# dansarie/sboxgates

Measured on NVIDIA H100. Metric: candidate 3-LUT tuples/sec on rijndael.txt --lut (T-units + C-units per second), higher is better.
Workload: dtype u32 bitwise (LOP3)

## Files before the change

### include/sboxgates_b200.h

```cpp
#ifndef SBOXGATES_B200_H
#define SBOXGATES_B200_H

#include <stdint.h>

#ifdef __cplusplus
extern "C" {
#endif

#define SBG_OK 0
#define SBG_ERR_ARG (-1)
#define SBG_ERR_CUDA (-2)
#define SBG_ERR_OVERFLOW (-3)
#define SBG_ERR_STATE (-4)

#define SBG_MAX_GATES 500
#define SBG_LIST_CAP 100000
#define SBG_KEY_NONE UINT64_MAX
#define SBG_PROBLEM_SLOTS 64
#define SBG_LANES 8

typedef struct sbg_handle sbg_handle;

typedef struct {
  int32_t found;
// ... 87 lines not shown
int sbg_enum7(sbg_handle *h, int part, int nparts, const uint8_t *outer_order,
    const uint8_t *middle_order, uint64_t max_matches, sbg_match *out, uint64_t *n_out,
    uint64_t *total, uint64_t *feasible);
int sbg_enum3(sbg_handle *h, int part, int nparts, const uint16_t *gate_order,
    uint64_t max_matches, sbg_match *out, uint64_t *n_out, uint64_t *total, uint64_t *feasible);

int sbg_enum_fetch(sbg_handle *h, uint64_t first, uint64_t count, sbg_match *out, uint64_t *n_out);
int sbg_enum_pick(sbg_handle *h, const uint64_t *ranks, uint64_t nranks, sbg_match *out);

int sbg_enum_block_sums(sbg_handle *h, uint64_t *out, uint64_t *nblocks);
int sbg_enum_set_global(sbg_handle *h, const uint64_t *sums, uint64_t stride,
    const uint64_t *counts, int nparts, uint64_t *total);

#define SBG_MAX_DEPTH 1020
#define SBG_DEPTH_BINS 1024
int sbg_enum_set_depth(sbg_handle *h, const uint16_t *depth, int n, uint32_t max_depth);
int sbg_enum_depth_counts(sbg_handle *h, uint64_t *out, uint32_t nbins);

int sbg_plan_tickets(int width, int prefix_gates, int n, uint32_t excluded, int mode,
                     uint64_t waves, uint64_t *out);

#define SBG_WEIGHTED_ROW 76
int sbg_weighted_tickets(int n, uint32_t group_pairs, uint32_t *out);

int sbg_ordering_row(int width, int k, int *row);
int sbg_solve_inner(const uint64_t *in1, const uint64_t *in2, const uint64_t *in3,
    const uint64_t *target, const uint64_t *mask, uint8_t *func, uint8_t *seen);
void sbg_lut_table(uint8_t func, const uint64_t *in1, const uint64_t *in2, const uint64_t *in3,
    uint64_t *out);

#ifdef __cplusplus
}
#endif
#endif
```

### sboxgates_b200/csrc/sbg_api.cu

```cuda
#include "sbg_device.cuh"

#include <algorithm>
#include <cstdarg>
#include <cstdio>
#include <cstdlib>
#include <cstring>
#include <ctime>
#include <map>
#include <type_traits>
#include <utility>
#include <vector>

#include "../../include/sboxgates_b200.h"

using namespace sbg;

namespace {


uint64_t h_binom[501][8];
int h_rows7[70][7];
int h_rows5[10][5];
bool g_tables_ready = false;

// ... 45 lines not shown
  for (int pos = 0; pos < t; pos++) {
    for (;; x++) {
      const uint64_t cnt = h_binom[n - x - 1][t - pos - 1];
      if (rank < cnt) break;
      rank -= cnt;
    }
    out[pos] = (uint16_t)x++;
  }
}

int popcount256(const uint64_t *m) {
  return __builtin_popcountll(m[0]) + __builtin_popcountll(m[1]) + __builtin_popcountll(m[2])
      + __builtin_popcountll(m[3]);
}

}


namespace {
constexpr int kSlots = SBG_PROBLEM_SLOTS;
constexpr int kLanes = SBG_LANES;
constexpr size_t kPerPrefixMax = SBG_LIST_CAP + 32 * 512;
constexpr size_t kPerChunkMax = 32 * 512;
constexpr size_t kDefaultHitsCap = (size_t)4 << 20;
constexpr size_t kGrownHitsCap = (size_t)32 << 20;
constexpr uint64_t kTicketTableMax = (uint64_t)1 << 24;
constexpr uint64_t kTicketSlack = 16384;
}

struct sbg_lane {
  cudaStream_t own_stream = nullptr;
  cudaStream_t stream = nullptr;
  DevCtl *d_ctl = nullptr;
  DevParams7 *d_par7 = nullptr;
  uint8_t *d_pos5 = nullptr;
  uint16_t *d_order3 = nullptr;
  HostOut *h_out = nullptr;
  HostOut *d_out = nullptr;
  DevCtl *h_ctl = nullptr;
  uint64_t *d_hits = nullptr;
  uint64_t *d_aux = nullptr;
  uint64_t *d_sorted = nullptr;
  uint32_t *d_tcount = nullptr;
  uint32_t *d_toffset = nullptr;
  uint32_t *d_gcount = nullptr;
  uint64_t *d_sieve3 = nullptr;
// ... 461 lines not shown
  const int n = hp.n;
  int mode = h->opt_head;
  if (mode < 0) {
    mode = n >= kHeadAlwaysMinGates || (hp.m <= kHeadMaxPositions && n >= kHeadMinGates) ? 1 : 0;
  }
  if (retry) mode = n >= kHeadAlwaysMinGates ? 2 : 0;
  const uint64_t qmax = P == 4 ? h_binom[n - 5][2] : (uint64_t)(n - 6);
  return plan_chunks_mode<P, 7>(n, hp.inmask, mode, kHeadWaves, qmax);
}

struct FilterPlan {
  ChunkPlan pl;
  uint64_t total = 0;
  uint64_t tickets = 0;
  uint64_t chunk_tickets = 0;
  uint64_t batch = 1;
  uint64_t ticket_bound = 0;
  uint64_t tickets_cap = 0;
  int max_warps = 0;
  bool five = false;
  uint64_t seg_base = 0;
  uint32_t list_base = 0;
  WeightedTickets wt;
};

void build_weighted(int n, uint32_t group_pairs, WeightedTickets *wt) {
  memset(wt, 0, sizeof *wt);
  const int np = n - 3;
  if (np < 4 || np >= kWeightedRow || group_pairs == 0) return;
  wt->group_pairs = group_pairs;
  uint64_t prev[kWeightedRow + 1] = {0}, cur[kWeightedRow + 1];
  for (int x = np - 1; x >= 0; x--) {
    const uint64_t r = (uint64_t)(n - x - 2);
    const uint64_t pairs = r >= 2 ? r * (r - 1) / 2 : 0;
    const uint64_t f = std::max<uint64_t>(1, (pairs + group_pairs - 1) / group_pairs);
    prev[x] = prev[x + 1] + f;
  }
  for (int x = 0; x < kWeightedRow; x++) wt->w[0][x] = (uint32_t)prev[x];
  for (int r = 2; r <= 4; r++) {
    memset(cur, 0, sizeof cur);
    for (int x = np - r; x >= 0; x--) cur[x] = cur[x + 1] + prev[x + 1];
    for (int x = 0; x < kWeightedRow; x++) wt->w[r - 1][x] = (uint32_t)cur[x];
    memcpy(prev, cur, sizeof cur);
  }
  wt->total = wt->w[3][0];
}

constexpr uint32_t kGroupChunks = 6;

template <int P>
FilterPlan plan_filter_p(const sbg_handle *h, const sbg_lane &L, const sbg_handle::HostProblem &hp,
    int nparts, bool retry, uint64_t seg_base) {
  FilterPlan fp;
  fp.seg_base = seg_base;
  const int n = hp.n;
  fp.five = P == 5;
  fp.total = h_binom[n - (7 - P)][P];
  fp.pl = plan_chunks<P>(h, hp, retry);
  fp.max_warps = !retry ? 0 : (int)std::max<size_t>(1, fp.pl.all
      ? (L.hits_cap - SBG_LIST_CAP) / kPerChunkMax : L.hits_cap / kPerPrefixMax - 1);
  fp.tickets = fp.pl.all ? 0 : (fp.total - fp.pl.t_offset + nparts - 1) / nparts;
  fp.chunk_tickets = (fp.pl.items + kDeal * nparts - 1) / (kDeal * nparts) * kDeal;
  fp.batch = fp.pl.all ? 1 : pick_batch(h, fp.tickets, n, P == 4 ? 4 : 6);
  if (fp.max_warps > 0) fp.batch = 1;
  fp.wt.group_pairs = 0;
  if (P == 4 && !retry && !h->concurrent && fp.pl.items == 0 && n >= 7 && n <= kWeightedMaxGates) {
    build_weighted(n, 32u * kGroupChunks, &fp.wt);
    if (fp.wt.group_pairs != 0) {
      fp.tickets = ((uint64_t)fp.wt.total + nparts - 1) / nparts;
      fp.batch = 1;
    }
  }
  fp.ticket_bound = fp.chunk_tickets + (fp.tickets + 2 * kDeal) / fp.batch + 2 + kTicketSlack;
  const uint64_t left = fp.ticket_bound > seg_base ? fp.ticket_bound - seg_base : kTicketSlack;
  fp.tickets_cap = std::min<uint64_t>(left, h->ticket_table_max + kTicketSlack);
  return fp;
}

bool filter_uses_five(const sbg_handle *h, int n) {
  return h->opt_pm_prefix != 0 ? h->opt_pm_prefix == 5 : n >= kPm5MinGates;
}

FilterPlan plan_filter(const sbg_handle *h, const sbg_lane &L, const sbg_handle::HostProblem &hp,
    int nparts, bool retry, uint64_t seg_base = 0) {
  return filter_uses_five(h, hp.n) ? plan_filter_p<5>(h, L, hp, nparts, retry, seg_base)
                                   : plan_filter_p<4>(h, L, hp, nparts, retry, seg_base);
}

template <int P>
int launch_filter7_pm_p(sbg_handle *h, sbg_lane &L, const FilterPlan &fp, int part, int nparts,
    unsigned long long list_cap, bool build_sieve3) {
  const sbg_handle::HostProblem &hp = h->slots[L.slot];
  const int n = hp.n;
  const int m = hp.m;
  const ChunkPlan &pl = fp.pl;
  const bool shifted = P == 4 && (h->opt_shift >= 0 ? h->opt_shift != 0 && n <= 63
                                                     : n <= kShiftMaxGates);
  const bool sieve = h->opt_sieve == 2 || (h->opt_sieve == 1 && m > kSieveMinPositions);
  return with_nw(hp.nw, [&](auto nw_c) {
    constexpr int NW = decltype(nw_c)::value;
    auto run = [&](auto kernel, bool sh, bool sv) {
      const size_t smem = filter_pm_smem<NW, P>(n, m, sh, sv);
      int rc;
      if ((rc = ensure_smem(h, kernel, smem)) != SBG_OK) return rc;
      int grid = grid_for(h, kernel, smem, fp.tickets + fp.chunk_tickets);
      if (fp.max_warps > 0) grid = std::min(grid, (fp.max_warps + kWarpsPerCta - 1) / kWarpsPerCta);
      const cudaError_t e = launch(h, kernel, grid, kThreads, smem, L.stream, !h->timing,
          h->d_slots + L.slot, L.d_ctl, L.d_hits, L.d_aux, L.d_tcount, L.d_gcount,
          (unsigned long long)L.hits_cap, (unsigned long long)fp.tickets_cap, part, nparts,
          list_cap, (int)fp.batch, fp.max_warps,
          pl.all ? (unsigned long long)fp.total : pl.t_offset, pl.items, std::max(1, pl.chunks),
          (unsigned long long)fp.chunk_tickets, (unsigned long long)fp.seg_base,
          h->opt_packed ? 15 : 0, fp.wt, (const uint64_t *)L.d_sieve3);
      if (e != cudaSuccess) return fail(h, SBG_ERR_CUDA, "k_filter7_pm: %s", cudaGetErrorString(e));
      return SBG_OK;
    };
    if constexpr (P == 4) {
      if (shifted && sieve) {
        if (build_sieve3) {
          int rc;
          if ((rc = ensure_sieve3(h, L, n)) != SBG_OK) return rc;
          const int grid = (int)((h_binom[n - 4][3] + kWarpsPerCta - 1) / kWarpsPerCta);
          const cudaError_t e = launch(h, k_sieve3<NW>, grid, kThreads, 0, L.stream, !h->timing,
              h->d_slots + L.slot, (const DevCtl *)L.d_ctl, L.d_sieve3);
          if (e != cudaSuccess) return fail(h, SBG_ERR_CUDA, "k_sieve3: %s", cudaGetErrorString(e));
        }
        return run(k_filter7_pm<NW, 1, P, true, true, true>, true, true);
      }
      if (shifted) return run(k_filter7_pm<NW, 1, P, true, true, false>, true, false);
    }
    if (n <= 31) return run(k_filter7_pm<NW, 1, P, true, false, false>, false, false);
    if (n <= 63) return run(k_filter7_pm<NW, 2, P, true, false, false>, false, false);
    return run(k_filter7_pm<NW, 2, P, false, false, false>, false, false);
  });
}

int enqueue_filter7(sbg_handle *h, sbg_lane &L, const FilterPlan &fp, int part, int nparts,
    bool build_sieve3) {
  int rc;
  if (h->timing) cudaEventRecord(L.ev[0], L.stream);
  const unsigned long long room = (unsigned long long)SBG_LIST_CAP - fp.list_base;
// ... 768 lines not shown
  build_host_tables();
  if (out == nullptr || n < width || n > SBG_MAX_GATES) return SBG_ERR_ARG;
  ChunkPlan pl;
  uint64_t total = 0;
  if (width == 7 && prefix_gates == 4 && n >= 8) {
    pl = plan_chunks_mode<4, 7>(n, excluded, mode, waves, h_binom[n - 5][2]);
    total = h_binom[n - 3][4];
  } else if (width == 7 && prefix_gates == 5 && n >= 8) {
    pl = plan_chunks_mode<5, 7>(n, excluded, mode, waves, (uint64_t)(n - 6));
    total = h_binom[n - 2][5];
  } else if (width == 5 && prefix_gates == 3 && n >= 8) {
    pl = plan_chunks_mode<3, 5>(n, excluded, mode, waves, h_binom[n - 3][2]);
    total = h_binom[n - 2][3];
  } else {
    return SBG_ERR_ARG;
  }
  out[0] = pl.items;
  out[1] = (uint64_t)pl.chunks;
  out[2] = pl.items == 0 ? 0 : (pl.all ? total : pl.t_offset);
  out[3] = total;
  return SBG_OK;
}

int sbg_weighted_tickets(int n, uint32_t group_pairs, uint32_t *out) {
  static_assert(SBG_WEIGHTED_ROW == kWeightedRow, "header and device code agree on the row length");
  if (out == nullptr || n < 7 || n > kWeightedMaxGates || group_pairs == 0) return SBG_ERR_ARG;
  WeightedTickets wt;
  build_weighted(n, group_pairs, &wt);
  if (wt.group_pairs == 0) return SBG_ERR_ARG;
  out[0] = wt.total;
  for (int r = 0; r < 4; r++) {
    for (int x = 0; x < kWeightedRow; x++) out[1 + kWeightedRow * r + x] = wt.w[r][x];
  }
  return SBG_OK;
}

int sbg_ordering_row(int width, int k, int *row) {
  build_host_tables();
  if (row == nullptr) return SBG_ERR_ARG;
  if (width == 5 && k >= 0 && k < 10) {
    for (int i = 0; i < 5; i++) row[i] = h_rows5[k][i];
    return SBG_OK;
  }
  if (width == 7 && k >= 0 && k < 70) {
    for (int i = 0; i < 7; i++) row[i] = h_rows7[k][i];
    return SBG_OK;
  }
  return SBG_ERR_ARG;
}

void sbg_lut_table(uint8_t func, const uint64_t *in1, const uint64_t *in2, const uint64_t *in3,
    uint64_t *out) {
  for (int v = 0; v < 4; v++) {
    uint64_t r = 0;
    for (int m = 0; m < 8; m++) {
// ... 989 lines not shown
```

### sboxgates_b200/csrc/sbg_device.cuh

```cuda
#pragma once

#if defined(SBG_COUNT_STAGE1) || defined(SBG_COUNT_FILTER) || defined(SBG_TIME_FILTER)
#include <cstdio>
#endif
#if defined(SBG_COUNT_FILTER) && defined(SBG_TIME_FILTER)
#error "SBG_COUNT_FILTER and SBG_TIME_FILTER share the control block's spare words"
#endif
#include <cuda_pipeline.h>
#include <cuda_runtime.h>
#include <stdint.h>

#include <type_traits>

namespace sbg {

constexpr int kMaxGatesPad = 512;
constexpr int kThreads = 256;
constexpr int kWarpsPerCta = kThreads / 32;
constexpr unsigned kFull = 0xffffffffu;
constexpr uint64_t kDeal = 16;

struct DevProblem {
  uint32_t tabs[8][kMaxGatesPad];
  uint32_t T[8];
// ... 595 lines not shown
      if (lane == 0) t = atomicAdd(&ctl->ticket2, 1ull);
      t = __shfl_sync(kFull, t, 0);
      if (t >= count) break;
      const uint64_t rank = hits[2 * t];
      if ((volatile_load(&ctl->best) >> 12) < rank) continue;
      const uint64_t packed = hits[2 * t + 1];
      int g5[5];
#pragma unroll
      for (int i = 0; i < 5; i++) g5[i] = (int)((packed >> (9 * (4 - i))) & 0x1ffu);
      const uint32_t hit = decomp5_tuple<NW>(s_tabs, npad, g5, T, M, lane, s_pos, tab);
      if (hit != 0xffffffffu && lane == 0) {
        atomicMin(&ctl->best, (unsigned long long)((rank << 12) | (uint64_t)hit));
      }
    }
  }
  let_successor_start();
  if (last_cta_of_grid(ctl) && threadIdx.x == 0 && !skip) {
    close_stage(ctl, out, 1, volatile_load(&ctl->best), count, 0, 0);
  }
}

constexpr int kWeightedMaxGates = 72;
constexpr int kWeightedRow = 76;
struct WeightedTickets {
  uint32_t group_pairs;
  uint32_t total;
  uint32_t w[4][kWeightedRow];
};

__device__ __forceinline__ void unrank_weighted_warp(uint32_t t, int np,
    const uint32_t (*__restrict__ w)[kWeightedRow], int *pre, uint32_t &group, int lane) {
  int x0 = 0;
#pragma unroll
  for (int pos = 0; pos < 4; pos++) {
    const int r = 4 - pos;
    const uint32_t *wr = w[r - 1];
    const uint32_t total = wr[x0];
    int cnt = 0;
    for (int y0 = x0;; y0 += 32) {
      const int y = y0 + lane;
      const bool le = y <= np - r && total - wr[min(y, kWeightedRow - 1)] <= t;
      const uint32_t bal = __ballot_sync(kFull, le);
      cnt += __popc(bal);
      if (bal != 0xffffffffu) break;
    }
    const int e = x0 + cnt - 1;
    t -= total - wr[e];
    pre[pos] = e;
    x0 = e + 1;
  }
  group = t;
}

#ifndef SBG_FILTER_MIN_CTAS
#define SBG_FILTER_MIN_CTAS (SH ? 3 : 2)
#endif
constexpr int kQuadGates = 7;
constexpr int kSievePairs = 64;
constexpr int kSieveWords = 4 * kSievePairs;

constexpr int kSieve3Words = 2 * kSievePairs;
template <int NW>
__global__ void __launch_bounds__(kThreads) k_sieve3(const DevProblem *__restrict__ prob,
    const DevCtl *__restrict__ ctl, uint64_t *__restrict__ table) {
  __shared__ uint64_t s_pairs[kWarpsPerCta][kSievePairs];
  __shared__ uint64_t s_rows[256];
  __shared__ uint32_t s_tabs[NW][64];
  __shared__ uint32_t s_T[NW], s_M[NW];
  wait_for_predecessor();
  if (chain_is_over(ctl) || volatile_load32(&ctl->skip7) != 0) return;
  const int n = prob->n;
  const int m = prob->m;
  const uint32_t inmask = prob->inmask;
  const int lane = threadIdx.x & 31;
// ... 78 lines not shown
      const uint32_t hi = npairs > 32 ? __ballot_sync(kFull, ((s_hi >> x) & 1u) != 0) : 0u;
      const uint64_t v = (((uint64_t)hi << 32) | lo) | unused;
      if (lane == (x & 31)) {
        if (x < 32) sep_lo = v;
        else sep_hi = v;
      }
    }
    uint64_t *e = table + t * kSieve3Words;
    e[lane] = s_lo;
    e[lane + 32] = s_hi;
    e[kSievePairs + lane] = sep_lo;
    e[kSievePairs + lane + 32] = sep_hi;
  }
}
template <int NW, int W, int P, bool FS, bool SH = false, bool SV = false>
__global__ void __launch_bounds__(kThreads, SBG_FILTER_MIN_CTAS) k_filter7_pm(const DevProblem *__restrict__ prob,
    DevCtl *__restrict__ ctl, uint64_t *__restrict__ hits, uint64_t *__restrict__ aux,
    uint32_t *__restrict__ tcount, uint32_t *__restrict__ gcount, unsigned long long hits_cap,
    unsigned long long tickets_cap, int part, int nparts, unsigned long long list_cap, int batch,
    int max_warps, unsigned long long t_offset, unsigned long long chunk_items,
    int chunks_per_prefix, unsigned long long chunk_tickets, unsigned long long seg_base,
    int packed_gates, const WeightedTickets wt, const uint64_t *__restrict__ sieve3) {
  constexpr int K = 7, NC = 1 << P, NP = P == 4 ? 4 : 2;
  extern __shared__ uint32_t smem[];
  __shared__ uint32_t s_wt[4][kWeightedRow];
  wait_for_predecessor();
  const int n = prob->n;
  const int m = prob->m;
  const int npad = (n + 3) & ~3;
  const int ngw = (((n + 31) >> 5) + 1) & ~1;
  uint32_t *s_tabs = smem;
  uint32_t *s_xr = smem + NW * npad;
  const int lane = threadIdx.x & 31;
  const int warp = threadIdx.x >> 5;
  uint32_t *cells = s_xr + ((m * ngw + 3) & ~3) + warp * (NC * NW);
  uint32_t *vs = s_xr + ((m * ngw + 3) & ~3) + kWarpsPerCta * (NC * NW) + warp * (ngw * 32);
  uint64_t *s_sieve = reinterpret_cast<uint64_t *>(s_xr + ((m * ngw + 3) & ~3)
      + kWarpsPerCta * (NC * NW + ngw * 32) + warp * kSieveWords);
  uint32_t *sxt = s_xr + ((m * ngw + 3) & ~3)
      + kWarpsPerCta * (NC * NW + ngw * 32 + (SV ? kSieveWords : 0));
  static_assert(!SH || (W == 1 && P == 4 && FS), "shifted windows: one word, 4-gate prefixes, n <= 63");
  static_assert(!SV || SH, "the sieve is part of the shifted-window form");
  const uint32_t sxt_top = (uint32_t)__cvta_generic_to_shared(sxt + 31);
  const uint32_t xr_base = (uint32_t)__cvta_generic_to_shared(s_xr);
  const uint32_t neg_row_bytes = 0u - (uint32_t)ngw * 4u;
  const uint32_t low31 = 0x7fffffffu ^ (((uint32_t)max_warps >> 31) & (uint32_t)lane);
// ... 74 lines not shown
      q_hc[i] = next_hc;
    }
  }
  for (;;) {
    if (!ahead) {
      fetch();
      q_b[0] = next_b;
      q_hc[0] = next_hc;
    }
    const unsigned long long b = __shfl_sync(kFull, q_b[0], 0);
    const unsigned long long hc_then = __shfl_sync(kFull, q_hc[0], 0);
    if (b >= tickets_cap) {
      if (lane == 0 && hc_then < list_cap) atomicMax(&ctl->overflow, 2u);
      break;
    }
    if (hc_then >= list_cap) {
      if (lane == 0) tcount[b] = 0;
      break;
    }
    uint32_t tj = 0;
    uint64_t t_first, t_end;
    uint32_t q_begin = 0, q_limit = 0xffffffffu;
    const unsigned long long bg = seg_base + b;
    const bool weighted = P == 4 && wt.group_pairs != 0;
    const bool chunked = !weighted && bg < chunk_tickets;
    const uint64_t lt = (chunked || weighted) ? bg : (bg - chunk_tickets) * (uint64_t)batch;
    const uint64_t dealt = dealt_item(lt, part, nparts);
    bool valid = true;
    if (weighted) {
      if (dealt >= (uint64_t)wt.total) {
        if (lane == 0) tcount[b] = 0;
        break;
      }
      t_first = 0;
      t_end = 1;
    } else if (chunked) {
      valid = dealt < chunk_items;
      t_first = dealt / (uint64_t)chunks_per_prefix;
      t_end = t_first + 1;
      q_begin = (uint32_t)(dealt % (uint64_t)chunks_per_prefix) * 32u;
      q_limit = q_begin + 32u;
    } else {
      t_first = t_offset + dealt;
      if (t_first >= total) {
        if (lane == 0) tcount[b] = 0;
        break;
      }
      t_end = min(t_first + (uint64_t)batch, total);
    }
    if (ahead) {
#pragma unroll
      for (int i = 0; i + 1 < kDepth; i++) {
        q_b[i] = q_b[i + 1];
        q_hc[i] = q_hc[i + 1];
      }
      fetch();
      q_b[kDepth - 1] = next_b;
      q_hc[kDepth - 1] = next_hc;
    }
    if (valid) {
    int pre[P];
    uint64_t unused_rank;
    if constexpr (P == 4) {
      if (weighted) {
        uint32_t group;
        unrank_weighted_warp((uint32_t)dealt, n - (K - P), s_wt, pre, group, lane);
        q_begin = group * wt.group_pairs;
        q_limit = q_begin + wt.group_pairs;
      }
    }
    if (!weighted) {
      unrank_prefix_warp<P, K, false>(t_first, chunked ? n_allowed : n, pre, unused_rank, lane);
    }
    if (chunked) {
#pragma unroll
      for (int i = 0; i < P; i++) {
        int g = pre[i];
#pragma unroll
        for (int bit = 0; bit < 8; bit++) g += (((inmask >> bit) & 1u) != 0 && bit <= g) ? 1 : 0;
        pre[i] = g;
      }
    }
    for (uint64_t gt = t_first; gt < t_end; gt++) {
      if (gt != t_first) {
        int i = P - 1;
        while (i > 0 && pre[i] + (P - i) >= n - (K - P)) i--;
        pre[i]++;
        for (int k2 = i + 1; k2 < P; k2++) pre[k2] = pre[k2 - 1] + 1;
      }
      const int last = pre[P - 1];
      const int r = n - last - 2;
      const uint32_t Q = P == 4 ? (uint32_t)(r * (r - 1) / 2) : (uint32_t)r;
      if (q_begin >= max(Q, 1u)) continue;
      bool rejected = false;
#pragma unroll
      for (int i = 0; i < P; i++) rejected |= (pre[i] < 8) && ((inmask >> pre[i]) & 1u);
      if (rejected) {
        if (q_begin == 0 && lane == 0) swept_lane += c_binom[n - last - 1][K - P];
        continue;
      }
      SBG_TF_MARK(0);

      auto find_mixed_cells = [&]() {
        constexpr bool kSplit = NC == 16 && NW >= 2;
        constexpr int NWH = kSplit ? NW / 2 : NW;
        const bool upper = kSplit && lane >= 16;
        const int cell = lane & (NC - 1);
        const uint32_t *tabs_h = s_tabs + (upper ? NWH * npad : 0);
        uint32_t c[NWH];
        uint32_t ones = 0, zeros = 0;
#pragma unroll
        for (int k = 0; k < NWH; k++) {
          const int wk = upper ? k + NWH : k;
          uint32_t tt = SV ? prob->M[wk] : upper ? M[kSplit ? k + NWH : k] : M[k];
          const uint32_t tw = SV ? prob->T[wk] : upper ? T[kSplit ? k + NWH : k] : T[k];
#pragma unroll
          for (int i = 0; i < P; i++) {
            const uint32_t tv = tabs_h[k * npad + pre[i]];
            tt &= ((cell >> (P - 1 - i)) & 1) ? tv : ~tv;
          }
          c[k] = tt;
          ones |= tt & tw;
          zeros |= tt & ~tw;
        }
        if (kSplit) {
          ones |= __shfl_xor_sync(kFull, ones, 16);
          zeros |= __shfl_xor_sync(kFull, zeros, 16);
        }
        const bool mixed = ones != 0 && zeros != 0;
        const uint32_t mixed_ballot = __ballot_sync(kFull, mixed)
            & (NC == 32 ? 0xffffffffu : ((1u << (NC & 31)) - 1u));
        __syncwarp();
        if (mixed) {
          const int slot = __popc(mixed_ballot & ((1u << cell) - 1u));
#pragma unroll
          for (int k = 0; k < NWH; k++) cells[slot * NW + (upper ? NWH : 0) + k] = c[k];
        }
        __syncwarp();
        return __popc(mixed_ballot);
      };
      int mc = SV ? -1 : find_mixed_cells();
      SBG_TF_MARK(1);
#ifdef SBG_COUNT_FILTER
      unsigned long long dbg_chunks = 0, dbg_windows = 0, dbg_cells = 0, dbg_pos = 0, dbg_packed = 0;
      unsigned long long dbg_quad = 0, dbg_sieve = 0, dbg_exact = 0;
      unsigned long long dbg_mc = SV ? 0ull : (unsigned long long)mc;
#endif
      if constexpr (SV) {
        const int abc = (pre[0] << 18) | (pre[1] << 9) | pre[2];
        if (abc != sieve_abc) {
          sieve_abc = abc;
          const uint64_t rank3 = c_binom[pre[2]][3] + c_binom[pre[1]][2] + (uint64_t)pre[0];
          const uint4 *src = reinterpret_cast<const uint4 *>(sieve3 + rank3 * kSieve3Words);
          uint4 *dst = reinterpret_cast<uint4 *>(s_sieve);
          const uint4 v0 = src[lane], v1 = src[lane + 32];
          __syncwarp();
          dst[lane] = v0;
          dst[lane + 32] = v1;
          __syncwarp();
        }
        SBG_TF_MARK(2);
      }

      unsigned long long emitted = 0;
      bool prefix_done = false;
      int run_i = 0, run_j = 1;
      if (P == 4 && q_begin + (uint32_t)lane < Q) unrank_pair(q_begin + (uint32_t)lane, r, run_i, run_j);
      for (uint32_t q0 = q_begin; q0 < min(Q, q_limit) && !prefix_done; q0 += 32) {
        const uint32_t q = q0 + lane;
        bool lane_ok = q < Q;
#ifdef SBG_COUNT_FILTER
        dbg_chunks++;
#endif
        int pi = 0, pj = 0;
        if (P == 4) {
          if (q0 != q_begin) {
            run_j += 32;
            while (run_j >= r && run_i < r - 2) {
              run_i++;
              run_j += run_i + 1 - r;
            }
          }
          pi = lane_ok ? run_i : 0;
          pj = lane_ok ? run_j : 1;
        } else {
          pj = lane_ok ? (int)q : 0;
        }
        const int ge = P == 4 ? last + 1 + pi : pre[P - 1];
        const int gf = last + 1 + pj;
        if (lane_ok) swept_lane += (unsigned long long)(n - 1 - gf);
        if (P == 4 && ge < 8 && ((inmask >> ge) & 1u)) lane_ok = false;
        if (gf < 8 && ((inmask >> gf) & 1u)) lane_ok = false;
        const uint32_t *tab_e = s_tabs + ge, *tab_f = s_tabs + gf;
        int first_g = last + (K - P);
        uint64_t cand = 0;
        if constexpr (SV) {
          if (lane_ok) cand = ((1ull << n) - 1u) & (~0ull << (gf + 1)) & ~(uint64_t)(inmask & 0xffu);
          {
            const uint64_t sepd = s_sieve[kSievePairs + pre[3]] | s_sieve[kSievePairs + ge]
                | s_sieve[kSievePairs + gf];
            uint32_t u_lo = ~(uint32_t)sepd, u_hi = ~(uint32_t)(sepd >> 32);
#ifdef SBG_COUNT_FILTER
            uint32_t its = 0;
#endif
            while ((u_lo | u_hi) != 0 && cand != 0) {
              const uint64_t s_a = u_lo != 0 ? s_sieve[__ffs(u_lo) - 1] : ~0ull;
              const uint64_t s_b = u_hi != 0 ? s_sieve[31 + __ffs(u_hi)] : ~0ull;
              cand &= s_a & s_b;
              u_lo &= u_lo - 1;
              u_hi &= u_hi - 1;
#ifdef SBG_COUNT_FILTER
              its++;
#endif
            }
#ifdef SBG_COUNT_FILTER
            dbg_sieve += __reduce_max_sync(kFull, its);
#endif
          }
          const uint32_t lo = __reduce_min_sync(kFull, cand != 0 ? (uint32_t)(__ffsll((long long)cand) - 1)
                                                                 : (uint32_t)n);
          SBG_TF_MARK(4);
          if (lo >= (uint32_t)n) continue;
          first_g = (int)lo;
          if (mc < 0) {
            mc = find_mixed_cells();
            SBG_TF_MARK(1);
#ifdef SBG_COUNT_FILTER
            dbg_mc = (unsigned long long)mc;
#endif
          }
#ifdef SBG_COUNT_FILTER
          dbg_exact++;
#endif
        } else if constexpr (SH) {
          const uint32_t lo = __reduce_min_sync(kFull, lane_ok ? (uint32_t)(gf + 1) : (uint32_t)n);
          if (lo >= (uint32_t)n) continue;
          first_g = (int)lo;
        }
        const int wb0 = SH ? 0 : ((first_g >> 5) & ~(W - 1));
        int nvw = 0;
        bool chunk_live = false;
        for (int wb = wb0; SH ? (first_g + 31 * wb < n) : (wb < ((n + 31) >> 5)); wb += W) {
          const int base = SH ? first_g + 31 * wb : 0;
          const bool packed = SH && n - base <= packed_gates;
          const bool quad = packed && n - base <= kQuadGates;
          const uint32_t sx_top = sxt_top + (uint32_t)((base - 6) * m) * 4u;
          uint32_t V[W];
          if constexpr (SV) {
            V[0] = (uint32_t)(cand >> base) & 0x7fffffffu;
          } else if constexpr (SH) {
            uint32_t v = 0x7fffffffu;
            if (n - base < 31) v = 0x7fffffffu >> (31 - (n - base));
            if (gf + 1 - base >= 31) v = 0u;
            else if (gf + 1 - base > 0) v &= 0xffffffffu << (gf + 1 - base);
            if (base < 8) v &= ~(inmask >> base);
            V[0] = lane_ok ? v : 0u;
          } else {
#pragma unroll
            for (int j = 0; j < W; j++) {
              const int g0 = (wb + j) * 32;
              uint32_t v = 0xffffffffu;
              if (n - g0 < 32) v = (n - g0 <= 0) ? 0u : (0xffffffffu >> (32 - (n - g0)));
              if (gf + 1 - g0 >= 32) v = 0u;
              else if (gf + 1 - g0 > 0) v &= 0xffffffffu << (gf + 1 - g0);
              if (g0 == 0) v &= ~inmask;
              V[j] = lane_ok ? v : 0u;
            }
          }
          bool alive = false;
#pragma unroll
          for (int j = 0; j < W; j++) alive |= V[j] != 0;
#ifdef SBG_COUNT_FILTER
// ... 132 lines not shown
                for (int k = 0; k < NP; k++) {
#pragma unroll
                  for (int jw = 0; jw < W; jw++) {
                    a_and[k][jw] = lop3<0xd0>(a_and[k][jw], x[jw], mk[k]);
                    a_or[k][jw] = lop3<0xf8>(a_or[k][jw], x[jw], mk[k]);
                  }
                }
              }
            }
#pragma unroll
            for (int k = 0; k < NP; k++) {
              const uint32_t both = FS
                  ? (uint32_t)((int32_t)(a_or[k][W - 1] & ~a_and[k][W - 1]) >> 31)
                  : (seen1[k] & seen0[k]);
#pragma unroll
              for (int jw = 0; jw < W; jw++) V[jw] &= a_and[k][jw] | ~a_or[k][jw] | ~both;
            }
            alive = false;
#pragma unroll
            for (int jw = 0; jw < W; jw++) alive |= V[jw] != 0;
            any_alive = __any_sync(kFull, alive);
          }
          chunk_live |= any_alive;
#pragma unroll
          for (int jw = 0; jw < W; jw++) vs[(nvw + jw) * 32 + lane] = V[jw];
          nvw += W;
        }
        SBG_TF_MARK(5);
        if (!chunk_live) continue;
        int cnt = 0;
        for (int i = 0; i < nvw; i++) cnt += __popc(vs[i * 32 + lane]);
        int incl = cnt;
#pragma unroll
        for (int d = 1; d < 32; d <<= 1) {
          const int up = __shfl_up_sync(kFull, incl, d);
          if (lane >= d) incl += up;
        }
        const int warp_total = __shfl_sync(kFull, incl, 31);
        unsigned long long base_slot = 0;
        if (lane == 0) base_slot = atomicAdd(&ctl->hit_count, (unsigned long long)warp_total);
        base_slot = __shfl_sync(kFull, base_slot, 0) + (unsigned long long)(incl - cnt);
        uint64_t where = (b << 22) | (uint64_t)(tj + (uint32_t)(incl - cnt));
        uint64_t head = 0;
#pragma unroll
        for (int i = 0; i < P; i++) head = (head << 9) | (uint64_t)pre[i];
        if (P == 4) {
          head = (head << 27) | ((uint64_t)ge << 18) | ((uint64_t)gf << 9);
        } else {
          head = (head << 18) | ((uint64_t)gf << 9);
        }
        if (cnt != 0) {
          for (int i = 0; i < nvw; i++) {
            uint32_t v = vs[i * 32 + lane];
            const int g0 = SH ? first_g + 31 * i : (wb0 + i) * 32;
            while (v != 0) {
              const int gbit = __ffs(v) - 1;
              v &= v - 1;
              if (base_slot < hits_cap) {
                hits[base_slot] = head | (uint64_t)(g0 + gbit);
                aux[base_slot] = where;
              } else {
                atomicExch(&ctl->overflow, 1u);
              }
              base_slot++;
              where++;
            }
          }
        }
// ... 37 lines not shown
constexpr int kTicketGroup = 1024;

__global__ void __launch_bounds__(256) k_offsets(DevCtl *__restrict__ ctl,
    const uint32_t *__restrict__ tcount, const uint32_t *__restrict__ gcount,
    uint32_t *__restrict__ toffset, unsigned long long tickets_cap, unsigned int list_cap,
    unsigned int list_base) {
  __shared__ unsigned long long s_part[8];
  __shared__ uint32_t s_scan[8];
  wait_for_predecessor();
  if (chain_is_over(ctl) || volatile_load32(&ctl->skip7) != 0) return;
  const unsigned long long handed = min(volatile_load(&ctl->ticket), tickets_cap);
  const unsigned long long first = (unsigned long long)blockIdx.x * kTicketGroup;
  if (blockIdx.x == 0 && threadIdx.x == 0) {
    const unsigned long long total = (unsigned long long)list_base
        + min(volatile_load(&ctl->hit_count), (unsigned long long)0xffffffffu);
    ctl->list_count = (unsigned int)min(total, (unsigned long long)list_cap);
#ifdef SBG_COUNT_FILTER
    printf("F1 prefixes %llu chunks %llu windows %llu cells %llu positions %llu packed %llu mixed %llu hits %llu quad %llu sieve %llu exact %llu\n",
        ctl->pad1[0], ctl->pad1[1], ctl->pad1[2], ctl->pad1[3], ctl->pad1[4], ctl->pad1[5],
        ctl->pad1[6], ctl->hit_count, ctl->pad1[7], ctl->pad1[8], ctl->pad1[9]);
    for (int i = 0; i < 10; i++) ctl->pad1[i] = 0;
#endif
#ifdef SBG_TIME_FILTER
    printf("T1 ticket %llu mixed %llu pairs %llu sep %llu sieve %llu cells %llu emit %llu\n",
        ctl->pad1[0], ctl->pad1[1], ctl->pad1[2], ctl->pad1[3], ctl->pad1[4], ctl->pad1[5],
        ctl->pad1[6]);
    for (int i = 0; i < 7; i++) ctl->pad1[i] = 0;
#endif
  }
  if (first >= handed) return;
  unsigned long long before = 0;
  for (unsigned int g = threadIdx.x; g < blockIdx.x; g += blockDim.x) before += gcount[g];
#pragma unroll
  for (int d = 16; d > 0; d >>= 1) before += __shfl_xor_sync(kFull, before, d);
  if ((threadIdx.x & 31) == 0) s_part[threadIdx.x >> 5] = before;
  __syncthreads();
  before = list_base;
#pragma unroll
  for (int i = 0; i < 8; i++) before += s_part[i];
  const unsigned long long t0 = first + 4ull * threadIdx.x;
  uint32_t c[4];
#pragma unroll
  for (int i = 0; i < 4; i++) c[i] = t0 + i < handed ? tcount[t0 + i] : 0u;
  const uint32_t mine = c[0] + c[1] + c[2] + c[3];
  uint32_t incl = mine;
#pragma unroll
  for (int d = 1; d < 32; d <<= 1) {
// ... 1521 lines not shown
```

### sboxgates_b200/native.py

```python
import ctypes as C
import os

import numpy as np

_HERE = os.path.dirname(os.path.abspath(__file__))
LIB_PATH = os.environ.get("SBG_LIB") or os.path.join(_HERE, "libsboxgates_b200.so")

SBG_OK = 0
SBG_LIST_CAP = 100000
SBG_KEY_NONE = (1 << 64) - 1


class NativeLibraryError(RuntimeError):
    pass


class SbgResult(C.Structure):
    _fields_ = [
        ("found", C.c_int32), ("ordering", C.c_int32), ("pos_outer", C.c_int32),
        ("pos_middle", C.c_int32), ("func_outer", C.c_uint8), ("func_middle", C.c_uint8),
        ("func_inner", C.c_uint8), ("inner_seen", C.c_uint8), ("gates", C.c_uint16 * 7),
        ("stale_outer", C.c_uint16), ("index", C.c_uint64), ("key", C.c_uint64),
        ("tuples_feasible", C.c_uint64), ("tuples_swept", C.c_uint64),
    ]
# ... 20 lines not shown
                        ("func_middle", "u1"), ("func_inner", "u1"), ("inner_seen", "u1"),
                        ("width", "u1"), ("pad", "u1", (5,))])
SBG_ENUM_MAX_MATCHES = 1 << 24
SBG_MAX_GATES = 500
SBG_MAX_DEPTH = 1020
SBG_DEPTH_BINS = 1024

SBG_DO_SCAN3, SBG_DO_SEARCH5, SBG_DO_SEARCH7 = 1, 2, 4
SBG_LANES = 8

u64p = C.POINTER(C.c_uint64)
u8p = C.POINTER(C.c_uint8)
i8p = C.POINTER(C.c_int8)

SIGNATURES = {
    "sbg_create": (C.c_int, [C.POINTER(C.c_void_p), C.c_int]),
    "sbg_destroy": (None, [C.c_void_p]),
    "sbg_last_error": (C.c_char_p, [C.c_void_p]),
    "sbg_set_stream": (C.c_int, [C.c_void_p, C.c_void_p]),
    "sbg_launch_count": (C.c_uint64, [C.c_void_p]),
    "sbg_plan_tickets": (C.c_int, [C.c_int, C.c_int, C.c_int, C.c_uint32, C.c_int, C.c_uint64,
                                   C.POINTER(C.c_uint64)]),
    "sbg_weighted_tickets": (C.c_int, [C.c_int, C.c_uint32, C.POINTER(C.c_uint32)]),
    "sbg_last_kernel_ms": (C.c_float, [C.c_void_p, C.c_int]),
    "sbg_set_timing": (C.c_int, [C.c_void_p, C.c_int]),
    "sbg_transfer_stats": (C.c_int, [C.c_void_p, C.POINTER(C.c_uint64)]),
    "sbg_host_seconds": (C.c_int, [C.c_void_p, C.POINTER(C.c_double)]),
    "sbg_alu_peak": (C.c_int, [C.c_void_p, C.POINTER(C.c_double)]),
    "sbg_search_node": (C.c_int, [C.c_void_p, C.POINTER(SbgJob), C.POINTER(SbgNodeResult)]),
    "sbg_search_batch": (C.c_int, [C.c_void_p, C.c_int, C.POINTER(SbgJob),
                                   C.POINTER(SbgNodeResult)]),
    "sbg_list7_device": (C.c_int, [C.c_void_p, C.POINTER(C.c_void_p), C.POINTER(C.c_int)]),
    "sbg_allgather_merge7": (C.c_int, [C.POINTER(C.c_void_p), C.c_int, C.POINTER(C.c_int)]),
    "sbg_set_list7_device": (C.c_int, [C.c_void_p, C.c_void_p, C.c_uint64, C.POINTER(C.c_int),
                                       C.c_int]),
    "sbg_load_problem": (C.c_int, [C.c_void_p, u64p, C.c_int, u64p, u64p, i8p]),
    "sbg_stage_problem": (C.c_int, [C.c_void_p, C.c_int, u64p, C.c_int, u64p, u64p, i8p]),
    "sbg_use_problem": (C.c_int, [C.c_void_p, C.c_int]),
    "sbg_search5": (C.c_int, [C.c_void_p, u8p, C.POINTER(SbgResult)]),
    "sbg_search7": (C.c_int, [C.c_void_p, u8p, u8p, C.POINTER(SbgResult)]),
    "sbg_search5_part": (C.c_int, [C.c_void_p, C.c_int, C.c_int, u8p, u64p]),
    "sbg_finish5": (C.c_int, [C.c_void_p, C.c_uint64, u8p, C.POINTER(SbgResult)]),
    "sbg_filter7_part": (C.c_int, [C.c_void_p, C.c_int, C.c_int, u64p, C.POINTER(C.c_int)]),
    "sbg_set_list7": (C.c_int, [C.c_void_p, u64p, C.c_int]),
    "sbg_decomp7_part": (C.c_int, [C.c_void_p, C.c_int, C.c_int, u8p, u8p, u64p]),
    "sbg_finish7": (C.c_int, [C.c_void_p, C.c_uint64, u8p, u8p, C.POINTER(SbgResult)]),
# ... 44 lines not shown
```

Before: 178000 billion.

## Tile sieve filter over 3-gate prefixes and walk triples per warp

In the sieve path of the 4-prefix filter, tickets now unrank only a 3-gate prefix (a,b,c) with weighted ticket tables built for P=3. Each warp walks (d,e,f) triples with a new step_triple/unrank_triple_warp scheme and groups lanes by d in passes, recomputing mixed cells per d. This lets sieve work and the a,b,c setup be shared across many d values and balances tickets by weight. The cost is extra per-pass ballots and reductions, more complex resume and swept-count accounting around t_offset, and a retry hit-capacity bound sized per ticket.

```diff
diff --git a/include/sboxgates_b200.h b/include/sboxgates_b200.h
--- a/include/sboxgates_b200.h
+++ b/include/sboxgates_b200.h
@@ -133,6 +133,8 @@
 
 #define SBG_WEIGHTED_ROW 76
 int sbg_weighted_tickets(int n, uint32_t group_pairs, uint32_t *out);
+int sbg_weighted_tickets_p(int n, int prefix_gates, uint32_t group_items, uint32_t *out);
+int sbg_triple_walk(int r, uint32_t q_begin, int chunks, int32_t *out);
 
 int sbg_ordering_row(int width, int k, int *row);
 int sbg_solve_inner(const uint64_t *in1, const uint64_t *in2, const uint64_t *in3,
diff --git a/sboxgates_b200/csrc/sbg_api.cu b/sboxgates_b200/csrc/sbg_api.cu
--- a/sboxgates_b200/csrc/sbg_api.cu
+++ b/sboxgates_b200/csrc/sbg_api.cu
@@ -91,6 +91,7 @@
 constexpr int kLanes = SBG_LANES;
 constexpr size_t kPerPrefixMax = SBG_LIST_CAP + 32 * 512;
 constexpr size_t kPerChunkMax = 32 * 512;
+constexpr size_t kPerTicketMax = kGroupChunks * kPerChunkMax;
 constexpr size_t kDefaultHitsCap = (size_t)4 << 20;
 constexpr size_t kGrownHitsCap = (size_t)32 << 20;
 constexpr uint64_t kTicketTableMax = (uint64_t)1 << 24;
@@ -598,31 +599,38 @@
   uint64_t seg_base = 0;
   uint32_t list_base = 0;
   WeightedTickets wt;
+  bool sieve = false;
+  uint64_t head = 0;
+  uint64_t head_end = 0;
 };
 
-void build_weighted(int n, uint32_t group_pairs, WeightedTickets *wt) {
+void build_weighted(int n, int P, uint32_t group_pairs, WeightedTickets *wt) {
   memset(wt, 0, sizeof *wt);
-  const int np = n - 3;
-  if (np < 4 || np >= kWeightedRow || group_pairs == 0) return;
+  const int np = n - (7 - P);
+  if (np < P || np >= kWeightedRow || group_pairs == 0 || P < 3 || P > 4) return;
   wt->group_pairs = group_pairs;
   uint64_t prev[kWeightedRow + 1] = {0}, cur[kWeightedRow + 1];
   for (int x = np - 1; x >= 0; x--) {
-    const uint64_t r = (uint64_t)(n - x - 2);
-    const uint64_t pairs = r >= 2 ? r * (r - 1) / 2 : 0;
-    const uint64_t f = std::max<uint64_t>(1, (pairs + group_pairs - 1) / group_pairs);
+    const uint64_t items = h_binom[n - x - 2][6 - P];
+    const uint64_t f = std::max<uint64_t>(1, (items + group_pairs - 1) / group_pairs);
     prev[x] = prev[x + 1] + f;
   }
   for (int x = 0; x < kWeightedRow; x++) wt->w[0][x] = (uint32_t)prev[x];
-  for (int r = 2; r <= 4; r++) {
+  for (int r = 2; r <= P; r++) {
     memset(cur, 0, sizeof cur);
     for (int x = np - r; x >= 0; x--) cur[x] = cur[x + 1] + prev[x + 1];
     for (int x = 0; x < kWeightedRow; x++) wt->w[r - 1][x] = (uint32_t)cur[x];
     memcpy(prev, cur, sizeof cur);
   }
-  wt->total = wt->w[3][0];
-}
-
-constexpr uint32_t kGroupChunks = 6;
+  wt->total = wt->w[P - 1][0];
+}
+
+bool filter_shifted(const sbg_handle *h, int n) {
+  return h->opt_shift >= 0 ? h->opt_shift != 0 && n <= 63 : n <= kShiftMaxGates;
+}
+bool filter_uses_sieve(const sbg_handle *h, int n, int m) {
+  return filter_shifted(h, n) && (h->opt_sieve == 2 || (h->opt_sieve == 1 && m > kSieveMinPositions));
+}
 
 template <int P>
 FilterPlan plan_filter_p(const sbg_handle *h, const sbg_lane &L, const sbg_handle::HostProblem &hp,
@@ -633,18 +641,46 @@
   fp.five = P == 5;
   fp.total = h_binom[n - (7 - P)][P];
   fp.pl = plan_chunks<P>(h, hp, retry);
-  fp.max_warps = !retry ? 0 : (int)std::max<size_t>(1, fp.pl.all
-      ? (L.hits_cap - SBG_LIST_CAP) / kPerChunkMax : L.hits_cap / kPerPrefixMax - 1);
-  fp.tickets = fp.pl.all ? 0 : (fp.total - fp.pl.t_offset + nparts - 1) / nparts;
-  fp.chunk_tickets = (fp.pl.items + kDeal * nparts - 1) / (kDeal * nparts) * kDeal;
-  fp.batch = fp.pl.all ? 1 : pick_batch(h, fp.tickets, n, P == 4 ? 4 : 6);
-  if (fp.max_warps > 0) fp.batch = 1;
   fp.wt.group_pairs = 0;
-  if (P == 4 && !retry && !h->concurrent && fp.pl.items == 0 && n >= 7 && n <= kWeightedMaxGates) {
-    build_weighted(n, 32u * kGroupChunks, &fp.wt);
-    if (fp.wt.group_pairs != 0) {
-      fp.tickets = ((uint64_t)fp.wt.total + nparts - 1) / nparts;
-      fp.batch = 1;
+  fp.sieve = P == 4 && nparts == 1 && filter_uses_sieve(h, n, hp.m);
+  if (fp.sieve) {
+    build_weighted(n, 3, 32u * kGroupChunks, &fp.wt);
+    fp.head = std::min<uint64_t>(fp.wt.total, (fp.pl.items + kGroupChunks - 1) / kGroupChunks)
+        * kGroupChunks;
+    fp.head_end = 0;
+    if (fp.pl.all) {
+      fp.head_end = ~0ull;
+    } else if (fp.pl.items != 0) {
+      uint64_t t = fp.pl.t_offset;
+      int x = 0;
+      for (int pos = 0; pos < 4; pos++) {
+        for (;; x++) {
+          const uint64_t cnt = h_binom[n - 3 - x - 1][4 - pos - 1];
+          if (t < cnt) break;
+          t -= cnt;
+        }
+        fp.head_end = (fp.head_end << 9) | (uint64_t)x++;
+      }
+    }
+    fp.pl = ChunkPlan();
+    fp.max_warps = !retry ? 0 : (int)std::max<size_t>(1,
+        (L.hits_cap - SBG_LIST_CAP) / kPerTicketMax);
+    fp.tickets = (fp.head + fp.wt.total - fp.head / kGroupChunks + nparts - 1) / nparts;
+    fp.chunk_tickets = 0;
+    fp.batch = 1;
+  } else {
+    fp.max_warps = !retry ? 0 : (int)std::max<size_t>(1, fp.pl.all
+        ? (L.hits_cap - SBG_LIST_CAP) / kPerChunkMax : L.hits_cap / kPerPrefixMax - 1);
+    fp.tickets = fp.pl.all ? 0 : (fp.total - fp.pl.t_offset + nparts - 1) / nparts;
+    fp.chunk_tickets = (fp.pl.items + kDeal * nparts - 1) / (kDeal * nparts) * kDeal;
+    fp.batch = fp.pl.all ? 1 : pick_batch(h, fp.tickets, n, P == 4 ? 4 : 6);
+    if (fp.max_warps > 0) fp.batch = 1;
+    if (P == 4 && !retry && !h->concurrent && fp.pl.items == 0 && n >= 7 && n <= kWeightedMaxGates) {
+      build_weighted(n, 4, 32u * kGroupChunks, &fp.wt);
+      if (fp.wt.group_pairs != 0) {
+        fp.tickets = ((uint64_t)fp.wt.total + nparts - 1) / nparts;
+        fp.batch = 1;
+      }
     }
   }
   fp.ticket_bound = fp.chunk_tickets + (fp.tickets + 2 * kDeal) / fp.batch + 2 + kTicketSlack;
@@ -670,9 +706,7 @@
   const int n = hp.n;
   const int m = hp.m;
   const ChunkPlan &pl = fp.pl;
-  const bool shifted = P == 4 && (h->opt_shift >= 0 ? h->opt_shift != 0 && n <= 63
-                                                     : n <= kShiftMaxGates);
-  const bool sieve = h->opt_sieve == 2 || (h->opt_sieve == 1 && m > kSieveMinPositions);
+  const bool shifted = P == 4 && filter_shifted(h, n);
   return with_nw(hp.nw, [&](auto nw_c) {
     constexpr int NW = decltype(nw_c)::value;
     auto run = [&](auto kernel, bool sh, bool sv) {
@@ -685,14 +719,15 @@
           h->d_slots + L.slot, L.d_ctl, L.d_hits, L.d_aux, L.d_tcount, L.d_gcount,
           (unsigned long long)L.hits_cap, (unsigned long long)fp.tickets_cap, part, nparts,
           list_cap, (int)fp.batch, fp.max_warps,
-          pl.all ? (unsigned long long)fp.total : pl.t_offset, pl.items, std::max(1, pl.chunks),
+          fp.sieve ? (unsigned long long)fp.head_end : pl.all ? (unsigned long long)fp.total : pl.t_offset,
+          fp.sieve ? (unsigned long long)fp.head : pl.items, std::max(1, pl.chunks),
           (unsigned long long)fp.chunk_tickets, (unsigned long long)fp.seg_base,
           h->opt_packed ? 15 : 0, fp.wt, (const uint64_t *)L.d_sieve3);
       if (e != cudaSuccess) return fail(h, SBG_ERR_CUDA, "k_filter7_pm: %s", cudaGetErrorString(e));
       return SBG_OK;
     };
     if constexpr (P == 4) {
-      if (shifted && sieve) {
+      if (fp.sieve) {
         if (build_sieve3) {
           int rc;
           if ((rc = ensure_sieve3(h, L, n)) != SBG_OK) return rc;
@@ -1507,15 +1542,34 @@
   return SBG_OK;
 }
 
-int sbg_weighted_tickets(int n, uint32_t group_pairs, uint32_t *out) {
+int sbg_weighted_tickets_p(int n, int prefix_gates, uint32_t group_items, uint32_t *out) {
   static_assert(SBG_WEIGHTED_ROW == kWeightedRow, "header and device code agree on the row length");
-  if (out == nullptr || n < 7 || n > kWeightedMaxGates || group_pairs == 0) return SBG_ERR_ARG;
+  build_host_tables();
+  if (out == nullptr || n < 7 || n > kWeightedMaxGates || group_items == 0
+      || prefix_gates < 3 || prefix_gates > 4) return SBG_ERR_ARG;
   WeightedTickets wt;
-  build_weighted(n, group_pairs, &wt);
+  build_weighted(n, prefix_gates, group_items, &wt);
   if (wt.group_pairs == 0) return SBG_ERR_ARG;
   out[0] = wt.total;
   for (int r = 0; r < 4; r++) {
     for (int x = 0; x < kWeightedRow; x++) out[1 + kWeightedRow * r + x] = wt.w[r][x];
+  }
+  return SBG_OK;
+}
+
+int sbg_weighted_tickets(int n, uint32_t group_pairs, uint32_t *out) {
+  return sbg_weighted_tickets_p(n, 4, group_pairs, out);
+}
+
+int sbg_triple_walk(int r, uint32_t q_begin, int chunks, int32_t *out) {
+  if (out == nullptr || r < 3 || r > 64 || chunks < 1) return SBG_ERR_ARG;
+  for (int lane = 0; lane < 32; lane++) {
+    int i = 0, j = 1, k = 2;
+    step_triple(i, j, k, r, (int)q_begin + lane);
+    for (int c = 0; c < chunks; c++) {
+      if (c > 0) step_triple(i, j, k, r, 32);
+      out[c * 32 + lane] = k < r ? (i << 16) | (j << 8) | k : -1;
+    }
   }
   return SBG_OK;
 }
diff --git a/sboxgates_b200/csrc/sbg_device.cuh b/sboxgates_b200/csrc/sbg_device.cuh
--- a/sboxgates_b200/csrc/sbg_device.cuh
+++ b/sboxgates_b200/csrc/sbg_device.cuh
@@ -641,18 +641,20 @@
 
 constexpr int kWeightedMaxGates = 72;
 constexpr int kWeightedRow = 76;
+constexpr uint32_t kGroupChunks = 6;
 struct WeightedTickets {
   uint32_t group_pairs;
   uint32_t total;
   uint32_t w[4][kWeightedRow];
 };
 
+template <int P>
 __device__ __forceinline__ void unrank_weighted_warp(uint32_t t, int np,
     const uint32_t (*__restrict__ w)[kWeightedRow], int *pre, uint32_t &group, int lane) {
   int x0 = 0;
 #pragma unroll
-  for (int pos = 0; pos < 4; pos++) {
-    const int r = 4 - pos;
+  for (int pos = 0; pos < P; pos++) {
+    const int r = P - pos;
     const uint32_t *wr = w[r - 1];
     const uint32_t total = wr[x0];
     int cnt = 0;
@@ -669,6 +671,47 @@
     x0 = e + 1;
   }
   group = t;
+}
+
+__device__ __forceinline__ void unrank_triple_warp(uint32_t q, int r, int &i, int &j, int &k,
+    int lane) {
+  const uint32_t all = (uint32_t)binom_arith((uint32_t)r, 3);
+  const int x0 = lane + 1, x1 = lane + 33;
+  i = __popc(__ballot_sync(kFull, x0 <= r - 3 && all - (uint32_t)binom_arith((uint32_t)(r - x0), 3) <= q))
+      + __popc(__ballot_sync(kFull, x1 <= r - 3 && all - (uint32_t)binom_arith((uint32_t)(r - x1), 3) <= q));
+  q -= all - (uint32_t)binom_arith((uint32_t)(r - i), 3);
+  const int rr = r - 1 - i;
+  const uint32_t pairs = (uint32_t)(rr * (rr - 1) / 2);
+  const int y = __popc(__ballot_sync(kFull, x0 <= rr - 2 && pairs - (uint32_t)((rr - x0) * (rr - x0 - 1) / 2) <= q))
+      + __popc(__ballot_sync(kFull, x1 <= rr - 2 && pairs - (uint32_t)((rr - x1) * (rr - x1 - 1) / 2) <= q));
+  q -= pairs - (uint32_t)((rr - y) * (rr - y - 1) / 2);
+  j = i + 1 + y;
+  k = j + 1 + (int)q;
+}
+
+__host__ __device__ __forceinline__ void step_triple(int &i, int &j, int &k, int r, int s) {
+  int rr = r - 1 - i;
+  const int a = j - i - 1;
+  int p = a * (2 * rr - a - 1) / 2 + (k - j - 1) + s;
+  int np = rr * (rr - 1) / 2;
+  while (p >= np && i < r - 3) {
+    p -= np;
+    i++;
+    rr--;
+    np = rr * (rr - 1) / 2;
+  }
+  if (p >= np) {
+    j = r - 2;
+    k = r + (p - np);
+    return;
+  }
+  const float b = 2.0f * rr - 1.0f;
+  int x = (int)((b - sqrtf(fmaxf(b * b - 8.0f * (float)p, 0.0f))) * 0.5f);
+  x = x < 0 ? 0 : x > rr - 2 ? rr - 2 : x;
+  while (x > 0 && x * (2 * rr - x - 1) / 2 > p) x--;
+  while ((x + 1) * (2 * rr - x - 2) / 2 <= p) x++;
+  j = i + 1 + x;
+  k = j + 1 + (p - x * (2 * rr - x - 1) / 2);
 }
 
 #ifndef SBG_FILTER_MIN_CTAS
@@ -793,6 +836,7 @@
     int chunks_per_prefix, unsigned long long chunk_tickets, unsigned long long seg_base,
     int packed_gates, const WeightedTickets wt, const uint64_t *__restrict__ sieve3) {
   constexpr int K = 7, NC = 1 << P, NP = P == 4 ? 4 : 2;
+  constexpr int PT = SV ? 3 : P;
   extern __shared__ uint32_t smem[];
   __shared__ uint32_t s_wt[4][kWeightedRow];
   wait_for_predecessor();
@@ -913,13 +957,23 @@
     uint64_t t_first, t_end;
     uint32_t q_begin = 0, q_limit = 0xffffffffu;
     const unsigned long long bg = seg_base + b;
-    const bool weighted = P == 4 && wt.group_pairs != 0;
+    const bool weighted = SV || (P == 4 && wt.group_pairs != 0);
     const bool chunked = !weighted && bg < chunk_tickets;
     const uint64_t lt = (chunked || weighted) ? bg : (bg - chunk_tickets) * (uint64_t)batch;
     const uint64_t dealt = dealt_item(lt, part, nparts);
     bool valid = true;
+    uint64_t wticket = dealt;
+    uint32_t head_chunk = kGroupChunks;
+    if (SV) {
+      if (dealt < chunk_items) {
+        wticket = dealt / kGroupChunks;
+        head_chunk = (uint32_t)(dealt % kGroupChunks);
+      } else {
+        wticket = dealt - (chunk_items - chunk_items / kGroupChunks);
+      }
+    }
     if (weighted) {
-      if (dealt >= (uint64_t)wt.total) {
+      if (wticket >= (uint64_t)wt.total) {
         if (lane == 0) tcount[b] = 0;
         break;
       }
@@ -955,9 +1009,13 @@
     if constexpr (P == 4) {
       if (weighted) {
         uint32_t group;
-        unrank_weighted_warp((uint32_t)dealt, n - (K - P), s_wt, pre, group, lane);
+        unrank_weighted_warp<PT>((uint32_t)wticket, n - (K - PT), s_wt, pre, group, lane);
         q_begin = group * wt.group_pairs;
         q_limit = q_begin + wt.group_pairs;
+        if (head_chunk < kGroupChunks) {
+          q_begin += 32u * head_chunk;
+          q_limit = q_begin + 32u;
+        }
       }
     }
     if (!weighted) {
@@ -979,15 +1037,24 @@
         pre[i]++;
         for (int k2 = i + 1; k2 < P; k2++) pre[k2] = pre[k2 - 1] + 1;
       }
-      const int last = pre[P - 1];
+      const int last = pre[PT - 1];
       const int r = n - last - 2;
-      const uint32_t Q = P == 4 ? (uint32_t)(r * (r - 1) / 2) : (uint32_t)r;
+      const uint32_t Q = SV ? (uint32_t)binom_arith((uint32_t)r, 3)
+          : P == 4 ? (uint32_t)(r * (r - 1) / 2) : (uint32_t)r;
       if (q_begin >= max(Q, 1u)) continue;
       bool rejected = false;
 #pragma unroll
-      for (int i = 0; i < P; i++) rejected |= (pre[i] < 8) && ((inmask >> pre[i]) & 1u);
+      for (int i = 0; i < PT; i++) rejected |= (pre[i] < 8) && ((inmask >> pre[i]) & 1u);
       if (rejected) {
-        if (q_begin == 0 && lane == 0) swept_lane += c_binom[n - last - 1][K - P];
+        if (q_begin == 0 && lane == 0) {
+          if constexpr (SV) {
+            const uint64_t abc = ((uint64_t)pre[0] << 18) | ((uint64_t)pre[1] << 9) | (uint64_t)pre[2];
+            swept_lane += abc > (t_offset >> 9) ? c_binom[n - last - 1][K - PT]
+                : abc < (t_offset >> 9) ? 0ull : c_binom[n - (int)(t_offset & 0x1ffu)][K - 3];
+          } else {
+            swept_lane += c_binom[n - last - 1][K - PT];
+          }
+        }
         continue;
       }
       SBG_TF_MARK(0);
@@ -1030,12 +1097,12 @@
         __syncwarp();
         return __popc(mixed_ballot);
       };
-      int mc = SV ? -1 : find_mixed_cells();
+      int mc = SV ? 0 : find_mixed_cells();
       SBG_TF_MARK(1);
 #ifdef SBG_COUNT_FILTER
       unsigned long long dbg_chunks = 0, dbg_windows = 0, dbg_cells = 0, dbg_pos = 0, dbg_packed = 0;
       unsigned long long dbg_quad = 0, dbg_sieve = 0, dbg_exact = 0;
-      unsigned long long dbg_mc = SV ? 0ull : (unsigned long long)mc;
+      unsigned long long dbg_mc = (unsigned long long)mc;
 #endif
       if constexpr (SV) {
         const int abc = (pre[0] << 18) | (pre[1] << 9) | pre[2];
@@ -1055,16 +1122,26 @@
 
       unsigned long long emitted = 0;
       bool prefix_done = false;
-      int run_i = 0, run_j = 1;
-      if (P == 4 && q_begin + (uint32_t)lane < Q) unrank_pair(q_begin + (uint32_t)lane, r, run_i, run_j);
+      int run_i = 0, run_j = 1, run_k = 0;
+      if constexpr (SV) {
+        unrank_triple_warp(q_begin, r, run_k, run_i, run_j, lane);
+        step_triple(run_k, run_i, run_j, r, lane);
+      } else if (P == 4 && q_begin + (uint32_t)lane < Q) {
+        unrank_pair(q_begin + (uint32_t)lane, r, run_i, run_j);
+      }
       for (uint32_t q0 = q_begin; q0 < min(Q, q_limit) && !prefix_done; q0 += 32) {
         const uint32_t q = q0 + lane;
         bool lane_ok = q < Q;
 #ifdef SBG_COUNT_FILTER
         dbg_chunks++;
 #endif
-        int pi = 0, pj = 0;
-        if (P == 4) {
+        int pi = 0, pj = 0, pd = 0;
+        if (SV) {
+          if (q0 != q_begin) step_triple(run_k, run_i, run_j, r, 32);
+          pd = lane_ok ? run_k : 0;
+          pi = lane_ok ? run_i : 1;
+          pj = lane_ok ? run_j : 2;
+        } else if (P == 4) {
           if (q0 != q_begin) {
             run_j += 32;
             while (run_j >= r && run_i < r - 2) {
@@ -1077,9 +1154,14 @@
         } else {
           pj = lane_ok ? (int)q : 0;
         }
+        const int gd = SV ? last + 1 + pd : pre[3];
         const int ge = P == 4 ? last + 1 + pi : pre[P - 1];
         const int gf = last + 1 + pj;
-        if (lane_ok) swept_lane += (unsigned long long)(n - 1 - gf);
+        const bool d_out = SV && gd < 8 && ((inmask >> gd) & 1u);
+        if (lane_ok && !(d_out && (((uint64_t)sieve_abc << 9) | (uint64_t)gd) < t_offset)) {
+          swept_lane += (unsigned long long)(n - 1 - gf);
+        }
+        if (d_out) lane_ok = false;
         if (P == 4 && ge < 8 && ((inmask >> ge) & 1u)) lane_ok = false;
         if (gf < 8 && ((inmask >> gf) & 1u)) lane_ok = false;
         const uint32_t *tab_e = s_tabs + ge, *tab_f = s_tabs + gf;
@@ -1088,7 +1170,7 @@
         if constexpr (SV) {
           if (lane_ok) cand = ((1ull << n) - 1u) & (~0ull << (gf + 1)) & ~(uint64_t)(inmask & 0xffu);
           {
-            const uint64_t sepd = s_sieve[kSievePairs + pre[3]] | s_sieve[kSievePairs + ge]
+            const uint64_t sepd = s_sieve[kSievePairs + gd] | s_sieve[kSievePairs + ge]
                 | s_sieve[kSievePairs + gf];
             uint32_t u_lo = ~(uint32_t)sepd, u_hi = ~(uint32_t)(sepd >> 32);
 #ifdef SBG_COUNT_FILTER
@@ -1113,13 +1195,6 @@
           SBG_TF_MARK(4);
           if (lo >= (uint32_t)n) continue;
           first_g = (int)lo;
-          if (mc < 0) {
-            mc = find_mixed_cells();
-            SBG_TF_MARK(1);
-#ifdef SBG_COUNT_FILTER
-            dbg_mc = (unsigned long long)mc;
-#endif
-          }
 #ifdef SBG_COUNT_FILTER
           dbg_exact++;
 #endif
@@ -1131,6 +1206,21 @@
         const int wb0 = SH ? 0 : ((first_g >> 5) & ~(W - 1));
         int nvw = 0;
         bool chunk_live = false;
+        uint32_t todo = SV ? __ballot_sync(kFull, cand != 0) : 0u;
+        do {
+        bool in_pass = true;
+        if constexpr (SV) {
+          const int d_pass = (int)__reduce_min_sync(kFull, ((todo >> lane) & 1u) ? (uint32_t)gd : (uint32_t)n);
+          in_pass = ((todo >> lane) & 1u) != 0 && gd == d_pass;
+          todo &= ~__ballot_sync(kFull, in_pass);
+          pre[3] = d_pass;
+          mc = find_mixed_cells();
+          SBG_TF_MARK(1);
+#ifdef SBG_COUNT_FILTER
+          dbg_mc += (unsigned long long)mc;
+#endif
+        }
+        nvw = 0;
         for (int wb = wb0; SH ? (first_g + 31 * wb < n) : (wb < ((n + 31) >> 5)); wb += W) {
           const int base = SH ? first_g + 31 * wb : 0;
           const bool packed = SH && n - base <= packed_gates;
@@ -1138,7 +1228,7 @@
           const uint32_t sx_top = sxt_top + (uint32_t)((base - 6) * m) * 4u;
           uint32_t V[W];
           if constexpr (SV) {
-            V[0] = (uint32_t)(cand >> base) & 0x7fffffffu;
+            V[0] = in_pass ? (uint32_t)(cand >> base) & 0x7fffffffu : 0u;
           } else if constexpr (SH) {
             uint32_t v = 0x7fffffffu;
             if (n - base < 31) v = 0x7fffffffu >> (31 - (n - base));
@@ -1317,10 +1407,13 @@
             any_alive = __any_sync(kFull, alive);
           }
           chunk_live |= any_alive;
-#pragma unroll
-          for (int jw = 0; jw < W; jw++) vs[(nvw + jw) * 32 + lane] = V[jw];
+          if (in_pass || cand == 0) {
+#pragma unroll
+            for (int jw = 0; jw < W; jw++) vs[(nvw + jw) * 32 + lane] = V[jw];
+          }
           nvw += W;
         }
+        } while (todo != 0);
         SBG_TF_MARK(5);
         if (!chunk_live) continue;
         int cnt = 0;
@@ -1338,7 +1431,7 @@
         uint64_t where = (b << 22) | (uint64_t)(tj + (uint32_t)(incl - cnt));
         uint64_t head = 0;
 #pragma unroll
-        for (int i = 0; i < P; i++) head = (head << 9) | (uint64_t)pre[i];
+        for (int i = 0; i < P; i++) head = (head << 9) | (uint64_t)(SV && i == 3 ? gd : pre[i]);
         if (P == 4) {
           head = (head << 27) | ((uint64_t)ge << 18) | ((uint64_t)gf << 9);
         } else {
@@ -1422,7 +1515,7 @@
     for (int i = 0; i < 10; i++) ctl->pad1[i] = 0;
 #endif
 #ifdef SBG_TIME_FILTER
-    printf("T1 ticket %llu mixed %llu pairs %llu sep %llu sieve %llu cells %llu emit %llu\n",
+    printf("T1 ticket %llu mixed %llu copy %llu unused %llu sieve %llu cells %llu emit %llu\n",
         ctl->pad1[0], ctl->pad1[1], ctl->pad1[2], ctl->pad1[3], ctl->pad1[4], ctl->pad1[5],
         ctl->pad1[6]);
     for (int i = 0; i < 7; i++) ctl->pad1[i] = 0;
diff --git a/sboxgates_b200/native.py b/sboxgates_b200/native.py
--- a/sboxgates_b200/native.py
+++ b/sboxgates_b200/native.py
@@ -66,6 +66,8 @@
     "sbg_plan_tickets": (C.c_int, [C.c_int, C.c_int, C.c_int, C.c_uint32, C.c_int, C.c_uint64,
                                    C.POINTER(C.c_uint64)]),
     "sbg_weighted_tickets": (C.c_int, [C.c_int, C.c_uint32, C.POINTER(C.c_uint32)]),
+    "sbg_weighted_tickets_p": (C.c_int, [C.c_int, C.c_int, C.c_uint32, C.POINTER(C.c_uint32)]),
+    "sbg_triple_walk": (C.c_int, [C.c_int, C.c_uint32, C.c_int, C.POINTER(C.c_int32)]),
     "sbg_last_kernel_ms": (C.c_float, [C.c_void_p, C.c_int]),
     "sbg_set_timing": (C.c_int, [C.c_void_p, C.c_int]),
     "sbg_transfer_stats": (C.c_int, [C.c_void_p, C.POINTER(C.c_uint64)]),
```

After: 188400 billion (median of 6 runs). 1.06x the previous value.
